# Vchitect/Latte

Measured on NVIDIA H100. Metric: denoising-steps/sec Latte-XL/2 16x256x256 (CFG pair per step), higher is better.
Workload: dtype fp16

## Files before the change

latte_b200/csrc/gemm.cu:

```cuda
#include <cstdio>
#include "common.h"
#include "ptx.cuh"
#include "wgmma.cuh"

#include <cstdlib>

namespace b200 {

namespace {

constexpr int BM = 128;
constexpr int BK = 64;
constexpr int kThreads = 384;
constexpr int kProducerRegs = 40;
constexpr int kConsumerRegs = 232;

template <int BN, int EPI>
struct Cfg {
  static constexpr bool RESID = EPI == B200_EPI_GATE_RESIDUAL;
  static constexpr int A_BYTES = BM * BK * 2;
  static constexpr int B_BYTES = BN * BK * 2;
  static constexpr int STAGE_BYTES = A_BYTES + B_BYTES;
  static constexpr int BAR_BYTES = 256;
  static constexpr int STAGES_FIT = (232448 - BAR_BYTES - 1024) / STAGE_BYTES;
  static constexpr int STAGES = STAGES_FIT > 8 ? 8 : STAGES_FIT;
  static constexpr int BAR_OFF = STAGES * STAGE_BYTES;
  static constexpr int SMEM_BYTES = BAR_OFF + BAR_BYTES + 1024;
  static_assert(STAGE_BYTES % 1024 == 0, "stage must keep 1 KiB alignment");
  static_assert(SMEM_BYTES <= 232448, "exceeds the 227 KB per-CTA shared memory limit");
  static_assert(2 * STAGES <= BAR_BYTES / 8, "barrier area too small");
};

struct GemmDev {
  int M, N, K;
  int num_m, num_n;
  const float* bias;
  void* out16;
  const float* gate;
  long long gate_bs;
  int rows_per_batch;
  const float* row_add;
  int row_add_div, row_add_period;
  const uint16_t* add16;
  uint16_t* out16b;
  int conv_taps, conv_cblk, conv_h, conv_w, conv_bw, conv_bh;
  int conv_dx[9], conv_dy[9], conv_dz[9];
  float* resid;
  int streamk;
  unsigned long long* sk_flags;
};

__device__ __forceinline__ void flag_release(unsigned long long* f, unsigned long long v) {
  asm volatile("st.release.gpu.global.u64 [%0], %1;" ::"l"(f), "l"(v) : "memory");
}
__device__ __forceinline__ void flag_wait(const unsigned long long* f, unsigned long long want) {
  const long long t0 = clock64();
  while (true) {
    unsigned long long v;
    asm volatile("ld.acquire.gpu.global.u64 %0, [%1];" : "=l"(v) : "l"(f) : "memory");
    if (v == want) return;
    if (clock64() - t0 > 4000000000LL) __trap();
    __nanosleep(64);
  }
// ... 18 lines not shown
  __host__ __device__ bool next(int& tile, int& kb0, int& kb1) {
    if (wave < full_waves) {
      tile = wave * P + pair;
      ++wave;
      kb0 = 0;
      kb1 = num_kb;
      return tile < num_tiles;
    }
    if (u >= u_end) return false;
    const int t = static_cast<int>((u_end - 1) / num_kb);
    const long long t0 = static_cast<long long>(t) * num_kb;
    kb1 = static_cast<int>(u_end - t0);
    kb0 = u > t0 ? static_cast<int>(u - t0) : 0;
    tile = full_waves * P + t;
    u_end = t0 + kb0;
    return true;
  }
};

__device__ __forceinline__ float gelu_tanh_grad(float x) {
  const float k0 = 0.7978845608028654f, k1 = 0.044715f;
  const float x2 = x * x;
  float t;
  asm("tanh.approx.f32 %0, %1;" : "=f"(t) : "f"(k0 * fmaf(k1 * x2, x, x)));
  const float sech2 = fmaf(-t, t, 1.0f);
  return fmaf(0.5f * x * sech2, k0 * fmaf(3.0f * k1, x2, 1.0f), fmaf(0.5f, t, 0.5f));
}

__device__ __forceinline__ float resid_delta(float acc, float b, float gt, float ra, bool has_ra) {
  const float dv = __fmul_rn(gt, __fadd_rn(acc, b));
  return has_ra ? __fadd_rn(dv, ra) : dv;
}

constexpr int kEpiChunk = 8;
__device__ __forceinline__ void epi_chunk_fence() { __syncwarp(); }

__device__ __forceinline__ float gelu_tanh(float x) {
  const float u = 0.7978845608028654f * fmaf(0.044715f * x * x, x, x);
  float t;
  asm("tanh.approx.f32 %0, %1;" : "=f"(t) : "f"(u));
  const float hx = 0.5f * x;
  return fmaf(hx, t, hx);
}

template <int BN, int EPI, bool BF16, int MN>
__global__ void __cluster_dims__(2, 1, 1) __launch_bounds__(kThreads, 1)
gemm_kernel(const __grid_constant__ CUtensorMap tmA, const __grid_constant__ CUtensorMap tmB, const GemmDev p) {
  using C = Cfg<BN, EPI>;
  constexpr int TA = MN & 1, TB = MN >> 1;
  static_assert(MN == 0 || MN == 2 || MN == 3, "operand layouts: 0 forward, 2 dgrad, 3 wgrad");
  static_assert((BN / 8) % kEpiChunk == 0, "the epilogue chunks must tile the 8-column groups of a tile exactly");
  extern __shared__ uint8_t smem_raw[];
  uint8_t* smem = reinterpret_cast<uint8_t*>((reinterpret_cast<uintptr_t>(smem_raw) + 1023) & ~uintptr_t(1023));
  uint64_t* bars = reinterpret_cast<uint64_t*>(smem + C::BAR_OFF);
  uint64_t* full = bars;
  uint64_t* empty = bars + C::STAGES;

  const int warp = threadIdx.x >> 5;
  const int lane = threadIdx.x & 31;

  if (threadIdx.x == 0) {
    tma_prefetch_desc(&tmA);
    tma_prefetch_desc(&tmB);
    for (int i = 0; i < C::STAGES; ++i) {
      mbar_init(&full[i], 1);
      mbar_init(&empty[i], 4);
    }
    fence_mbar_init();
  }
  cluster_sync_all();
  pdl_launch_dependents();

  const uint32_t rank = cluster_ctarank();
  const int num_pair_m = (p.num_m + 1) / 2;
  const int num_tiles = num_pair_m * p.num_n;
  const int my_pair = blockIdx.x >> 1;
  const int num_pairs = gridDim.x >> 1;
  const int num_kb = p.K / BK;
  const bool streamk = C::RESID && p.streamk != 0;

  if (warp < 4) {
    setmaxnreg_dec<kProducerRegs>();
    if (threadIdx.x == 0) {
      pdl_wait();
      TileSched sched(my_pair, num_pairs, num_tiles, num_kb, streamk);
      int stage = 0;
      uint32_t phase = 0;
      int tile, kb0, kb1;
      while (sched.next(tile, kb0, kb1)) {
        const int m_blk = 2 * (tile / p.num_n) + static_cast<int>(rank), n_blk = tile % p.num_n;
        const int w_row0 = n_blk * BN + static_cast<int>(rank) * (BN / 2);
        for (int kb = kb0; kb < kb1; ++kb) {
          mbar_wait(&empty[stage], phase ^ 1);
          mbar_arrive_expect_tx(&full[stage], C::STAGE_BYTES);
          uint8_t* sa = smem + stage * C::STAGE_BYTES;
          if (MN == 0 && p.conv_taps > 0) {
// ... 2 lines not shown
            const int hw = p.conv_h * p.conv_w;
            const int img = pix0 / hw, rem = pix0 % hw;
            tma_load_4d(sa, &tmA, &full[stage], cb * BK, rem % p.conv_w + p.conv_dx[tap], rem / p.conv_w + p.conv_dy[tap],
                        img + p.conv_dz[tap]);
          } else if constexpr (TA) {
#pragma unroll
            for (int j = 0; j < BM / 64; ++j) tma_load_2d(sa + j * 8192, &tmA, &full[stage], m_blk * BM + j * 64, kb * BK);
          } else {
            tma_load_2d(sa, &tmA, &full[stage], kb * BK, m_blk * BM);
          }
          if constexpr (TB) {
            constexpr int per_cta = BN / 128;
#pragma unroll
            for (int j = 0; j < per_cta; ++j)
              tma_load_2d_mcast(sa + C::A_BYTES + (rank * per_cta + j) * 8192, &tmB, &full[stage], w_row0 + j * 64, kb * BK, 0x3);
          } else {
            tma_load_2d_mcast(sa + C::A_BYTES + rank * (C::B_BYTES / 2), &tmB, &full[stage], kb * BK, w_row0, 0x3);
          }
          if (++stage == C::STAGES) { stage = 0; phase ^= 1; }
        }
      }
    }
    __syncwarp();
  } else {
    setmaxnreg_inc<kConsumerRegs>();
    pdl_wait();
    const int wg = (warp >> 2) - 1;
    const int te = threadIdx.x & 127;
    const int w4 = te >> 5, g = lane >> 2, cq = lane & 3;
    const uint32_t empty_peer = mapa_u32(&empty[0], rank ^ 1u);
    int stage = 0;
    uint32_t phase = 0;
    float acc[BN / 2];
    TileSched sched(my_pair, num_pairs, num_tiles, num_kb, streamk);
    int tile, kb0, kb1;
    while (sched.next(tile, kb0, kb1)) {
      const int m0 = (2 * (tile / p.num_n) + static_cast<int>(rank)) * BM, n0 = (tile % p.num_n) * BN;
      int prev = -1;
      for (int kb = kb0; kb < kb1; ++kb) {
        mbar_wait(&full[stage], phase);
        const uint32_t sa = smem_u32(smem + stage * C::STAGE_BYTES), sb = sa + C::A_BYTES;
        wgmma_fence();
        const uint64_t da = gmma_desc(sa + wg * 8192, TA ? 8192 : 16, 1024, GMMA_LAYOUT_SW128);
        const uint64_t db = gmma_desc(sb, TB ? 8192 : 16, 1024, GMMA_LAYOUT_SW128);
#pragma unroll
        for (int k = 0; k < BK / 16; ++k)
          WgmmaSS<BN, TA, TB, BF16>::mma(acc, gmma_desc_advance(da, k * (TA ? 2048 : 32)),
                                         gmma_desc_advance(db, k * (TB ? 2048 : 32)), (kb != kb0 || k) ? 1u : 0u);
        wgmma_commit();
        wgmma_wait<1>();
        if (prev >= 0 && te == 0) {
          mbar_arrive(&empty[prev]);
          mbar_arrive_cluster(empty_peer + prev * 8);
        }
        prev = stage;
        if (++stage == C::STAGES) { stage = 0; phase ^= 1; }
      }
      wgmma_wait<0>();
      reg_fence(acc);
      if (te == 0) {
        mbar_arrive(&empty[prev]);
        mbar_arrive_cluster(empty_peer + prev * 8);
      }

      const int r0 = m0 + wg * 64 + w4 * 16 + g;
      if constexpr (C::RESID) {
        const bool first_seg = kb0 == 0;
        const bool partial = kb0 > 0 || kb1 < num_kb;
        unsigned long long* flag = nullptr;
        if (partial) flag = p.sk_flags + (static_cast<size_t>(tile - sched.full_waves * num_pairs) * 2 + rank) * 2 + wg;
        if (kb0 > 0) {
          if (te == 0) {
            flag_wait(flag, static_cast<unsigned long long>(kb0));
            if (kb1 == num_kb) flag_release(flag, 0ull);
          }
          asm volatile("bar.sync %0, 128;" ::"r"(1 + wg) : "memory");
        }
        const float* bias = (p.bias && first_seg) ? p.bias : nullptr;
        const int live = (p.N - n0) / 8 < BN / 8 ? (p.N - n0) / 8 : BN / 8;
#pragma unroll
        for (int h = 0; h < 2; ++h) {
          const int row = r0 + 8 * h;
          const bool row_ok = row < p.M;
          if (BN > 192 && !row_ok) continue;
          const int prow = row_ok ? row : p.M - 1;
          const float* gate_row = p.gate + static_cast<long long>(prow / p.rows_per_batch) * p.gate_bs;
          const float* add_row = (p.row_add && first_seg) ? p.row_add + static_cast<size_t>((prow / p.row_add_div) % p.row_add_period) * p.N : nullptr;
          float* xrow = p.resid + static_cast<size_t>(prow) * p.N;
          if (BN <= 192 && live == BN / 8) {
#pragma unroll
            for (int j0 = 0; j0 < BN / 8; j0 += kEpiChunk) {
              float2 x[kEpiChunk];
#pragma unroll
              for (int j = 0; j < kEpiChunk; ++j)
                if (row_ok) x[j] = *reinterpret_cast<const float2*>(xrow + n0 + 8 * (j0 + j) + 2 * cq);
#pragma unroll
              for (int j = 0; j < kEpiChunk; ++j) {
                if (!row_ok) continue;
                const int col = n0 + 8 * (j0 + j) + 2 * cq;
                const float2 b2 = bias ? __ldg(reinterpret_cast<const float2*>(bias + col)) : make_float2(0.f, 0.f);
                const float2 gt = __ldg(reinterpret_cast<const float2*>(gate_row + col));
                const float2 ra = add_row ? __ldg(reinterpret_cast<const float2*>(add_row + col)) : make_float2(0.f, 0.f);
                x[j].x = __fadd_rn(x[j].x, resid_delta(acc[4 * (j0 + j) + 2 * h], b2.x, gt.x, ra.x, add_row != nullptr));
                x[j].y = __fadd_rn(x[j].y, resid_delta(acc[4 * (j0 + j) + 2 * h + 1], b2.y, gt.y, ra.y, add_row != nullptr));
                *reinterpret_cast<float2*>(xrow + col) = x[j];
              }
              epi_chunk_fence();
            }
          } else if (row_ok) {
#pragma unroll
            for (int j = 0; j < BN / 8; ++j) {
              if (j >= live) break;
              const int col = n0 + 8 * j + 2 * cq;
              const float2 b2 = bias ? __ldg(reinterpret_cast<const float2*>(bias + col)) : make_float2(0.f, 0.f);
              const float2 gt = __ldg(reinterpret_cast<const float2*>(gate_row + col));
              const float2 ra = add_row ? __ldg(reinterpret_cast<const float2*>(add_row + col)) : make_float2(0.f, 0.f);
              float2 x = *reinterpret_cast<const float2*>(xrow + col);
              x.x = __fadd_rn(x.x, resid_delta(acc[4 * j + 2 * h], b2.x, gt.x, ra.x, add_row != nullptr));
              x.y = __fadd_rn(x.y, resid_delta(acc[4 * j + 2 * h + 1], b2.y, gt.y, ra.y, add_row != nullptr));
              *reinterpret_cast<float2*>(xrow + col) = x;
            }
          }
        }
        if (partial && kb1 < num_kb) {
          __threadfence();
          asm volatile("bar.sync %0, 128;" ::"r"(1 + wg) : "memory");
          if (te == 0) flag_release(flag, static_cast<unsigned long long>(kb1));
        }
      } else {
        bool done = false;
        if constexpr (EPI == B200_EPI_BIAS || EPI == B200_EPI_BIAS_GELU) {
          if (p.N - n0 >= BN) {
            const bool row_ok[2] = {r0 < p.M, r0 + 8 < p.M};
            uint32_t* orow[2];
#pragma unroll
            for (int h = 0; h < 2; ++h)
              orow[h] = reinterpret_cast<uint32_t*>(reinterpret_cast<uint16_t*>(p.out16) + static_cast<size_t>(r0 + 8 * h) * p.N);
#pragma unroll
            for (int j0 = 0; j0 < BN / 8; j0 += kEpiChunk) {
              float2 b[kEpiChunk];
#pragma unroll
              for (int j = 0; j < kEpiChunk; ++j)
                b[j] = p.bias ? __ldg(reinterpret_cast<const float2*>(p.bias + n0 + 8 * (j0 + j) + 2 * cq)) : make_float2(0.f, 0.f);
#pragma unroll
              for (int h = 0; h < 2; ++h) {
                if (!row_ok[h]) continue;
#pragma unroll
                for (int j = 0; j < kEpiChunk; ++j) {
                  const int col = n0 + 8 * (j0 + j) + 2 * cq;
                  float f0 = acc[4 * (j0 + j) + 2 * h], f1 = acc[4 * (j0 + j) + 2 * h + 1];
                  if (p.bias) { f0 += b[j].x; f1 += b[j].y; }
                  if constexpr (EPI == B200_EPI_BIAS_GELU) { f0 = gelu_tanh(f0); f1 = gelu_tanh(f1); }
                  orow[h][col / 2] = pack2<BF16>(f0, f1);
                }
              }
              epi_chunk_fence();
            }
            done = true;
          }
        }
        if (!done) {
#pragma unroll
          for (int h = 0; h < 2; ++h) {
            const int row = r0 + 8 * h;
            if (row >= p.M) continue;
            uint32_t* orow = reinterpret_cast<uint32_t*>(reinterpret_cast<uint16_t*>(p.out16) + static_cast<size_t>(row) * p.N);
            const int live = (p.N - n0) / 8 < BN / 8 ? (p.N - n0) / 8 : BN / 8;
#pragma unroll
            for (int j = 0; j < BN / 8; ++j) {
              if (j >= live) break;
              const int col = n0 + 8 * j + 2 * cq;
              float f0 = acc[4 * j + 2 * h], f1 = acc[4 * j + 2 * h + 1];
              if (p.bias) {
                const float2 b = __ldg(reinterpret_cast<const float2*>(p.bias + col));
                f0 += b.x; f1 += b.y;
              }
              if constexpr (EPI == B200_EPI_BIAS_GELU) { f0 = gelu_tanh(f0); f1 = gelu_tanh(f1); }
              uint32_t val = pack2<BF16>(f0, f1);
              const size_t off = (static_cast<size_t>(row) * p.N + col) / 2;
              if constexpr (EPI == B200_EPI_BIAS_MUL16) {
                const float2 a = unpack2<BF16>(val), r = unpack2<BF16>(__ldg(reinterpret_cast<const uint32_t*>(p.add16) + off));
                val = pack2<BF16>(a.x * r.x, a.y * r.y);
              }
              if constexpr (EPI == B200_EPI_MUL_GELUGRAD16) {
                const float2 a = unpack2<BF16>(val), r = unpack2<BF16>(__ldg(reinterpret_cast<const uint32_t*>(p.add16) + off));
                val = pack2<BF16>(a.x * gelu_tanh_grad(r.x), a.y * gelu_tanh_grad(r.y));
              }
              if constexpr (EPI == B200_EPI_BIAS_GELU_BOTH) {
                const float2 a = unpack2<BF16>(val);
                reinterpret_cast<uint32_t*>(p.out16b)[off] = pack2<BF16>(gelu_tanh(a.x), gelu_tanh(a.y));
              }
              if constexpr (EPI == B200_EPI_BIAS_ADD16) {
                const float2 a = unpack2<BF16>(val), r = unpack2<BF16>(__ldg(reinterpret_cast<const uint32_t*>(p.add16) + off));
                val = pack2<BF16>(a.x + r.x, a.y + r.y);
              }
              orow[col / 2] = val;
            }
          }
        }
      }
    }
  }

  cluster_sync_all();
}

template <int BN, int EPI, bool BF16, int MN>
int launch_one(const CUtensorMap& tmA, const CUtensorMap& tmB, const GemmDev& p, int grid, cudaStream_t stream) {
  using C = Cfg<BN, EPI>;
  auto kern = gemm_kernel<BN, EPI, BF16, MN>;
  B200_SET_SMEM_ONCE(kern, C::SMEM_BYTES);
  B200_CHECK_CUDA(launch_pdl(kern, dim3(grid), dim3(kThreads), C::SMEM_BYTES, stream, tmA, tmB, p));
  return B200_OK;
}

template <int BN, bool BF16>
int launch_epi(int epi, int mn, const CUtensorMap& tmA, const CUtensorMap& tmB, const GemmDev& p, int grid, cudaStream_t s) {
  if (mn == 0) {
    switch (epi) {
      case B200_EPI_BIAS: return launch_one<BN, B200_EPI_BIAS, BF16, 0>(tmA, tmB, p, grid, s);
      case B200_EPI_BIAS_GELU: return launch_one<BN, B200_EPI_BIAS_GELU, BF16, 0>(tmA, tmB, p, grid, s);
      case B200_EPI_GATE_RESIDUAL: return launch_one<BN, B200_EPI_GATE_RESIDUAL, BF16, 0>(tmA, tmB, p, grid, s);
      case B200_EPI_BIAS_ADD16: return launch_one<BN, B200_EPI_BIAS_ADD16, BF16, 0>(tmA, tmB, p, grid, s);
      case B200_EPI_BIAS_MUL16: return launch_one<BN, B200_EPI_BIAS_MUL16, BF16, 0>(tmA, tmB, p, grid, s);
      case B200_EPI_BIAS_GELU_BOTH: return launch_one<BN, B200_EPI_BIAS_GELU_BOTH, BF16, 0>(tmA, tmB, p, grid, s);
      case B200_EPI_MUL_GELUGRAD16: return launch_one<BN, B200_EPI_MUL_GELUGRAD16, BF16, 0>(tmA, tmB, p, grid, s);
    }
  }
  if constexpr (BN != 192) {
    if (mn == 2 && epi == B200_EPI_BIAS) return launch_one<BN, B200_EPI_BIAS, BF16, 2>(tmA, tmB, p, grid, s);
    if (mn == 2 && epi == B200_EPI_MUL_GELUGRAD16) return launch_one<BN, B200_EPI_MUL_GELUGRAD16, BF16, 2>(tmA, tmB, p, grid, s);
    if (mn == 3 && epi == B200_EPI_GATE_RESIDUAL) return launch_one<BN, B200_EPI_GATE_RESIDUAL, BF16, 3>(tmA, tmB, p, grid, s);
  }
  set_error("gemm: epilogue %d with operand layout %d and block_n %d is not built", epi, mn, BN);
  return B200_ERR_UNSUPPORTED;
}

template <int BN>
int launch_bn(int bf16, int epi, int mn, const CUtensorMap& tmA, const CUtensorMap& tmB, const GemmDev& p, int grid,
              cudaStream_t s) {
  return bf16 ? launch_epi<BN, true>(epi, mn, tmA, tmB, p, grid, s) : launch_epi<BN, false>(epi, mn, tmA, tmB, p, grid, s);
}

constexpr int kStreamKMinKb = 32;
constexpr int kSkFlags = B200_GEMM_SK_FLAGS;

int streamk_min_kb() {
  static const int v = env_int("B200_GEMM_SK_MINKB", kStreamKMinKb);
  return v;
}


int pick_block_n(int M, int N, int K, bool resid, int sms) {
  if (N <= 128) return 128;
  static const bool no_sk = env_int("B200_GEMM_NO_STREAMK", 0) != 0;
  const bool sk = resid && !no_sk && K / BK >= streamk_min_kb();
  const int cand[3] = {256, 192, 128};
  int best = 128;
  double best_cost = 1e300;
  for (int i = 0; i < 3; ++i) {
    const long long tiles = static_cast<long long>((M + BM - 1) / BM) * ((N + cand[i] - 1) / cand[i]);
    const double waves = (sk && tiles > sms) ? static_cast<double>(tiles) / sms : static_cast<double>((tiles + sms - 1) / sms);
    const double cost = waves * (128 + cand[i] / 2);
    if (cost < best_cost - 1e-9) { best_cost = cost; best = cand[i]; }
  }
  return best;
}

struct GemmPlan { int bn, pairs, pair_tiles, num_kb, streamk; };
GemmPlan plan_gemm(int M, int N, int K, bool resid, int block_n, int sms, bool split_small = false) {
  static const bool no_sk = env_int("B200_GEMM_NO_STREAMK", 0) != 0;
  GemmPlan g;
  g.bn = block_n ? block_n : pick_block_n(M, N, K, resid, sms);
  const int num_m = (M + BM - 1) / BM, num_n = (N + g.bn - 1) / g.bn;
// ... 57 lines not shown
  const bool resid = a.epilogue == B200_EPI_GATE_RESIDUAL;
  if (resid) {
    B200_REQUIRE(a.resid && a.gate && a.rows_per_batch > 0, B200_ERR_SHAPE, "gemm: gated-residual epilogue needs resid, gate, rows_per_batch");
    B200_REQUIRE((reinterpret_cast<uintptr_t>(a.resid) & 15) == 0 && (reinterpret_cast<uintptr_t>(a.gate) & 15) == 0 &&
                     (a.gate_batch_stride % 4) == 0,
                 B200_ERR_ALIGN, "gemm: resid/gate must be 16-byte aligned");
    B200_REQUIRE(!a.row_add || (reinterpret_cast<uintptr_t>(a.row_add) & 15) == 0, B200_ERR_ALIGN, "gemm: row_add must be 16-byte aligned");
  } else {
    B200_REQUIRE(a.out16 && (reinterpret_cast<uintptr_t>(a.out16) & 15) == 0, B200_ERR_ALIGN, "gemm: out16 must be 16-byte aligned");
  }
  B200_REQUIRE(!a.bias || (reinterpret_cast<uintptr_t>(a.bias) & 15) == 0, B200_ERR_ALIGN, "gemm: bias must be 16-byte aligned");
  B200_TRY(check_arch());
  int sms = 0;
  B200_TRY(device_sm_count(&sms));

  B200_REQUIRE(a.block_n == 0 || a.block_n == 128 || a.block_n == 192 || a.block_n == 256, B200_ERR_UNSUPPORTED,
               "gemm: block_n must be 128, 192 or 256 (got %d)", a.block_n);
  int block_n = a.block_n;
  if (a.mn_major) {
    B200_REQUIRE((a.mn_major == 2 || a.mn_major == 3) && a.conv_taps == 0 && (!(a.mn_major & 1) || a.M % 8 == 0) &&
                     (!(a.mn_major & 2) || a.N % 128 == 0) && (a.block_n == 0 || a.block_n == 128 || a.block_n == 256),
                 B200_ERR_UNSUPPORTED, "gemm (transposed operands): mn_major 2 or 3, M %% 8 == 0, N %% 128 == 0, block_n 128 or 256 (M=%d N=%d)",
                 a.M, a.N);
    if (block_n == 0) {
      block_n = pick_block_n(a.M, a.N, a.K, a.epilogue == B200_EPI_GATE_RESIDUAL, sms);
      if (block_n == 192) block_n = (a.N % 256 == 0 || a.N > 1024) ? 256 : 128;
      static const int wgrad_bn = env_int("B200_WGRAD_BN", 0);
      if (a.mn_major == 3) block_n = (wgrad_bn == 128 || wgrad_bn == 256) ? wgrad_bn : (a.N >= 256 ? 256 : block_n);
    }
  }
  const GemmPlan plan = plan_gemm(a.M, a.N, a.K, a.epilogue == B200_EPI_GATE_RESIDUAL, block_n, sms, a.mn_major == 3);
  const int bn = plan.bn;

  CUtensorMap tmA, tmB;
  int conv_bw = 0, conv_bh = 0;
  {
    if (a.conv_taps > 0) {
      B200_REQUIRE(a.conv_taps <= 9 && a.conv_c % BK == 0 && a.K == a.conv_taps * a.conv_c &&
                       a.M == a.conv_n * a.conv_h * a.conv_w,
                   B200_ERR_SHAPE, "conv: inconsistent geometry (taps %d, C %d, K %d, M %d)", a.conv_taps, a.conv_c, a.K, a.M);
      conv_bw = a.conv_w >= BM ? BM : a.conv_w;
      conv_bh = BM / conv_bw;
      B200_REQUIRE(BM % conv_bw == 0 && a.conv_w % conv_bw == 0 && a.conv_h % conv_bh == 0, B200_ERR_UNSUPPORTED,
                   "conv: %dx%d feature map cannot be tiled by 128-pixel patches", a.conv_h, a.conv_w);
      const uint64_t dimsA[4] = {static_cast<uint64_t>(a.conv_c), static_cast<uint64_t>(a.conv_w), static_cast<uint64_t>(a.conv_h),
                                 static_cast<uint64_t>(a.conv_n)};
      const uint64_t strA[3] = {static_cast<uint64_t>(a.conv_c) * 2, static_cast<uint64_t>(a.conv_c) * 2 * a.conv_w,
                                static_cast<uint64_t>(a.conv_c) * 2 * a.conv_w * a.conv_h};
      const uint32_t boxA[4] = {BK, static_cast<uint32_t>(conv_bw), static_cast<uint32_t>(conv_bh), 1};
      B200_TRY(make_tmap_16bit(&tmA, a.A, 4, dimsA, strA, boxA, TMAP_SW_128));
    } else if (a.mn_major & 1) {
      const uint64_t dimsA[2] = {static_cast<uint64_t>(a.M), static_cast<uint64_t>(a.K)};
      const uint64_t strA[1] = {static_cast<uint64_t>(a.M) * 2};
      const uint32_t boxA[2] = {64, BK};
      B200_TRY(make_tmap_16bit(&tmA, a.A, 2, dimsA, strA, boxA, TMAP_SW_128));
    } else {
      const uint64_t dimsA[2] = {static_cast<uint64_t>(a.K), static_cast<uint64_t>(a.M)};
      const uint64_t strA[1] = {static_cast<uint64_t>(a.K) * 2};
      const uint32_t boxA[2] = {BK, BM};
      B200_TRY(make_tmap_16bit(&tmA, a.A, 2, dimsA, strA, boxA, TMAP_SW_128));
    }
    if (a.mn_major & 2) {
      const uint64_t dimsB[2] = {static_cast<uint64_t>(a.N), static_cast<uint64_t>(a.K)};
      const uint64_t strB[1] = {static_cast<uint64_t>(a.N) * 2};
      const uint32_t boxB[2] = {64, BK};
      B200_TRY(make_tmap_16bit(&tmB, a.W, 2, dimsB, strB, boxB, TMAP_SW_128));
    } else {
      const uint64_t dimsB[2] = {static_cast<uint64_t>(a.K), static_cast<uint64_t>(a.N)};
      const uint64_t strB[1] = {static_cast<uint64_t>(a.K) * 2};
      const uint32_t boxB[2] = {BK, static_cast<uint32_t>(bn / 2)};
      B200_TRY(make_tmap_16bit(&tmB, a.W, 2, dimsB, strB, boxB, TMAP_SW_128));
    }
  }
  GemmDev p;
  p.M = a.M; p.N = a.N; p.K = a.K;
  p.num_m = (a.M + BM - 1) / BM;
  p.num_n = (a.N + bn - 1) / bn;
  p.bias = a.bias;
  p.out16 = a.out16;
  p.gate = a.gate;
  p.gate_bs = a.gate_batch_stride;
  p.rows_per_batch = a.rows_per_batch > 0 ? a.rows_per_batch : 1;
  p.row_add = a.row_add;
  p.row_add_div = a.row_add_div > 0 ? a.row_add_div : 1;
  p.row_add_period = a.row_add_period > 0 ? a.row_add_period : 1;
  p.add16 = static_cast<const uint16_t*>(a.add16);
  p.out16b = static_cast<uint16_t*>(a.out16b);
  p.conv_taps = a.conv_taps;
  p.conv_cblk = a.conv_taps > 0 ? a.conv_c / BK : 0;
  p.conv_h = a.conv_h; p.conv_w = a.conv_w; p.conv_bw = conv_bw; p.conv_bh = conv_bh;
  for (int i = 0; i < 9; ++i) { p.conv_dx[i] = a.conv_dx[i]; p.conv_dy[i] = a.conv_dy[i]; p.conv_dz[i] = a.conv_dz[i]; }
  p.resid = a.resid;
  const int pair_tiles = plan.pair_tiles;
  const int grid = 2 * plan.pairs;
  {
    const int pairs = plan.pairs;
    const int streamed = pair_tiles % pairs + pairs;
    p.streamk = (plan.streamk && a.sk_flags != nullptr && streamed * 4 <= kSkFlags) ? 1 : 0;
    p.sk_flags = p.streamk ? a.sk_flags : nullptr;
  }
  switch (bn) {
    case 128: return launch_bn<128>(a.bf16, a.epilogue, a.mn_major, tmA, tmB, p, grid, stream);
    case 192: return launch_bn<192>(a.bf16, a.epilogue, a.mn_major, tmA, tmB, p, grid, stream);
    default: return launch_bn<256>(a.bf16, a.epilogue, a.mn_major, tmA, tmB, p, grid, stream);
  }
}

}
```

latte_b200/csrc/ptx.cuh:

```cuda
#pragma once
#include <cuda.h>
#include <cuda_runtime.h>
#include <cuda_fp16.h>
#include <cuda_bf16.h>
#include <cstdint>
#include <cstdio>

namespace b200 {

#ifndef B200_HANG_CYCLES
#define B200_HANG_CYCLES (4000000000ll)
#endif

__device__ __forceinline__ uint32_t smem_u32(const void* p) {
  return static_cast<uint32_t>(__cvta_generic_to_shared(p));
}
__device__ __forceinline__ uint32_t lane_id() { return threadIdx.x & 31; }

__device__ __forceinline__ void pdl_wait() { asm volatile("griddepcontrol.wait;" ::: "memory"); }
__device__ __forceinline__ void pdl_launch_dependents() { asm volatile("griddepcontrol.launch_dependents;" ::: "memory"); }

__device__ __forceinline__ void mbar_init(uint64_t* bar, uint32_t count) {
  asm volatile("mbarrier.init.shared::cta.b64 [%0], %1;" ::"r"(smem_u32(bar)), "r"(count) : "memory");
}
// ... 42 lines not shown
    }
  }
}

__device__ __forceinline__ bool mbar_try_wait_cluster(uint64_t* bar, uint32_t parity) {
  uint32_t ok;
  asm volatile(
      "{\n\t.reg .pred p;\n\t"
      "mbarrier.try_wait.parity.acquire.cluster.shared::cta.b64 p, [%1], %2;\n\t"
      "selp.u32 %0, 1, 0, p;\n\t}"
      : "=r"(ok)
      : "r"(smem_u32(bar)), "r"(parity)
      : "memory");
  return ok != 0;
}
__device__ __forceinline__ void mbar_wait_cluster(uint64_t* bar, uint32_t parity) {
  if (mbar_try_wait_cluster(bar, parity)) return;
  long long t0 = clock64();
  while (!mbar_try_wait_cluster(bar, parity)) {
    if (clock64() - t0 > B200_HANG_CYCLES) {
      __trap();
    }
  }
}

template <uint32_t N>
__device__ __forceinline__ void setmaxnreg_dec() { asm volatile("setmaxnreg.dec.sync.aligned.u32 %0;" ::"n"(N)); }
template <uint32_t N>
__device__ __forceinline__ void setmaxnreg_inc() { asm volatile("setmaxnreg.inc.sync.aligned.u32 %0;" ::"n"(N)); }

__device__ __forceinline__ void fence_proxy_async_smem() {
  asm volatile("fence.proxy.async.shared::cta;" ::: "memory");
}

__device__ __forceinline__ void tma_prefetch_desc(const CUtensorMap* m) {
  asm volatile("prefetch.tensormap [%0];" ::"l"(reinterpret_cast<uint64_t>(m)) : "memory");
}
__device__ __forceinline__ void tma_load_2d(void* dst, const CUtensorMap* m, uint64_t* bar, int c0, int c1) {
  asm volatile(
      "cp.async.bulk.tensor.2d.shared::cluster.global.tile.mbarrier::complete_tx::bytes [%0], [%1, {%3, %4}], [%2];"
      ::"r"(smem_u32(dst)), "l"(reinterpret_cast<uint64_t>(m)), "r"(smem_u32(bar)), "r"(c0), "r"(c1)
      : "memory");
}
__device__ __forceinline__ void tma_load_3d(void* dst, const CUtensorMap* m, uint64_t* bar, int c0, int c1, int c2) {
  asm volatile(
      "cp.async.bulk.tensor.3d.shared::cluster.global.tile.mbarrier::complete_tx::bytes [%0], [%1, {%3, %4, %5}], [%2];"
      ::"r"(smem_u32(dst)), "l"(reinterpret_cast<uint64_t>(m)), "r"(smem_u32(bar)), "r"(c0), "r"(c1), "r"(c2)
      : "memory");
}
__device__ __forceinline__ void tma_load_4d(void* dst, const CUtensorMap* m, uint64_t* bar, int c0, int c1, int c2,
                                            int c3) {
  asm volatile(
      "cp.async.bulk.tensor.4d.shared::cluster.global.tile.mbarrier::complete_tx::bytes [%0], [%1, {%3, %4, %5, %6}], [%2];"
      ::"r"(smem_u32(dst)), "l"(reinterpret_cast<uint64_t>(m)), "r"(smem_u32(bar)), "r"(c0), "r"(c1), "r"(c2), "r"(c3)
      : "memory");
}

__device__ __forceinline__ void tma_load_2d_mcast(void* dst, const CUtensorMap* m, uint64_t* bar, int c0, int c1,
                                                  uint16_t mask) {
  asm volatile(
      "cp.async.bulk.tensor.2d.shared::cluster.global.tile.mbarrier::complete_tx::bytes.multicast::cluster"
      " [%0], [%1, {%3, %4}], [%2], %5;"
      ::"r"(smem_u32(dst)), "l"(reinterpret_cast<uint64_t>(m)), "r"(smem_u32(bar)), "r"(c0), "r"(c1), "h"(mask)
      : "memory");
}

// ... 3 lines not shown
  return r;
}
__device__ __forceinline__ void mbar_arrive_cluster(uint32_t bar_cluster_addr) {
  asm volatile("mbarrier.arrive.shared::cluster.b64 _, [%0];" ::"r"(bar_cluster_addr) : "memory");
}
__device__ __forceinline__ uint32_t cluster_ctarank() {
  uint32_t r;
  asm volatile("mov.u32 %0, %%cluster_ctarank;" : "=r"(r));
  return r;
}
__device__ __forceinline__ void cluster_sync_all() {
  asm volatile("barrier.cluster.arrive.release.aligned;\n\tbarrier.cluster.wait.acquire.aligned;" ::: "memory");
}

__device__ __forceinline__ void tma_store_2d(const CUtensorMap* m, const void* src, int c0, int c1) {
  asm volatile("cp.async.bulk.tensor.2d.global.shared::cta.bulk_group [%0, {%2, %3}], [%1];"
               ::"l"(reinterpret_cast<uint64_t>(m)), "r"(smem_u32(src)), "r"(c0), "r"(c1)
               : "memory");
}
__device__ __forceinline__ void tma_store_3d(const CUtensorMap* m, const void* src, int c0, int c1, int c2) {
  asm volatile("cp.async.bulk.tensor.3d.global.shared::cta.bulk_group [%0, {%2, %3, %4}], [%1];"
               ::"l"(reinterpret_cast<uint64_t>(m)), "r"(smem_u32(src)), "r"(c0), "r"(c1), "r"(c2)
               : "memory");
}
__device__ __forceinline__ void tma_store_4d(const CUtensorMap* m, const void* src, int c0, int c1, int c2, int c3) {
  asm volatile("cp.async.bulk.tensor.4d.global.shared::cta.bulk_group [%0, {%2, %3, %4, %5}], [%1];"
               ::"l"(reinterpret_cast<uint64_t>(m)), "r"(smem_u32(src)), "r"(c0), "r"(c1), "r"(c2), "r"(c3)
               : "memory");
}
__device__ __forceinline__ void tma_reduce_add_2d(const CUtensorMap* m, const void* src, int c0, int c1) {
  asm volatile("cp.reduce.async.bulk.tensor.2d.global.shared::cta.add.tile.bulk_group [%0, {%2, %3}], [%1];"
               ::"l"(reinterpret_cast<uint64_t>(m)), "r"(smem_u32(src)), "r"(c0), "r"(c1)
               : "memory");
}
__device__ __forceinline__ void tma_store_commit() { asm volatile("cp.async.bulk.commit_group;" ::: "memory"); }
template <int N>
__device__ __forceinline__ void tma_store_wait_read() {
  asm volatile("cp.async.bulk.wait_group.read %0;" ::"n"(N) : "memory");
}
template <int N>
__device__ __forceinline__ void tma_store_wait_all() {
  asm volatile("cp.async.bulk.wait_group %0;" ::"n"(N) : "memory");
}

enum : uint32_t { GMMA_LAYOUT_NONE = 0, GMMA_LAYOUT_SW128 = 1, GMMA_LAYOUT_SW64 = 2, GMMA_LAYOUT_SW32 = 3 };

__device__ __forceinline__ uint64_t gmma_desc(uint32_t saddr, uint32_t lbo_bytes, uint32_t sbo_bytes, uint32_t layout) {
  uint64_t d = 0;
  d |= static_cast<uint64_t>((saddr >> 4) & 0x3FFF);
  d |= static_cast<uint64_t>((lbo_bytes >> 4) & 0x3FFF) << 16;
  d |= static_cast<uint64_t>((sbo_bytes >> 4) & 0x3FFF) << 32;
  d |= static_cast<uint64_t>(layout) << 62;
  return d;
}
__device__ __forceinline__ uint64_t gmma_desc_advance(uint64_t desc, uint32_t bytes) {
  return desc + static_cast<uint64_t>(bytes >> 4);
}
__device__ __forceinline__ void wgmma_fence() { asm volatile("wgmma.fence.sync.aligned;" ::: "memory"); }
__device__ __forceinline__ void wgmma_commit() { asm volatile("wgmma.commit_group.sync.aligned;" ::: "memory"); }
template <int N>
__device__ __forceinline__ void wgmma_wait() { asm volatile("wgmma.wait_group.sync.aligned %0;" ::"n"(N) : "memory"); }
template <int N>
__device__ __forceinline__ void reg_fence(float (&d)[N]) {
#pragma unroll
  for (int i = 0; i < N; ++i) asm volatile("" : "+f"(d[i])::"memory");
}
// ... 22 lines not shown
```

Baseline: 39.48.

## Stage GEMM epilogues through swizzled shared memory and TMA store/reduce-add

Replaces the per-thread direct global stores in the GEMM epilogue with staging into double-buffered 128B-swizzled shared memory (stmatrix for 16-bit outputs, st.shared for fp32 residual deltas). The tile is then written out by a TMA bulk store, or by a TMA reduce-add into the fp32 residual stream instead of a read-modify-write. The aim is coalesced, asynchronous output traffic and removal of the residual read. In exchange, 32 KB of shared memory goes to epilogue buffers, which can cut pipeline stages. It also adds two named barriers per chunk and changes stream-K ordering to rely on async-proxy fences.

```diff
diff --git a/latte_b200/csrc/gemm.cu b/latte_b200/csrc/gemm.cu
--- a/latte_b200/csrc/gemm.cu
+++ b/latte_b200/csrc/gemm.cu
@@ -14,6 +14,8 @@
 constexpr int kThreads = 384;
 constexpr int kProducerRegs = 40;
 constexpr int kConsumerRegs = 232;
+
+constexpr int kEpiBufBytes = 64 * 128;
 
 template <int BN, int EPI>
 struct Cfg {
@@ -21,14 +23,17 @@
   static constexpr int A_BYTES = BM * BK * 2;
   static constexpr int B_BYTES = BN * BK * 2;
   static constexpr int STAGE_BYTES = A_BYTES + B_BYTES;
+  static constexpr int EPI_BYTES = 2 * 2 * kEpiBufBytes;
   static constexpr int BAR_BYTES = 256;
-  static constexpr int STAGES_FIT = (232448 - BAR_BYTES - 1024) / STAGE_BYTES;
+  static constexpr int STAGES_FIT = (232448 - EPI_BYTES - BAR_BYTES - 1024) / STAGE_BYTES;
   static constexpr int STAGES = STAGES_FIT > 8 ? 8 : STAGES_FIT;
-  static constexpr int BAR_OFF = STAGES * STAGE_BYTES;
+  static constexpr int EPI_OFF = STAGES * STAGE_BYTES;
+  static constexpr int BAR_OFF = EPI_OFF + EPI_BYTES;
   static constexpr int SMEM_BYTES = BAR_OFF + BAR_BYTES + 1024;
   static_assert(STAGE_BYTES % 1024 == 0, "stage must keep 1 KiB alignment");
   static_assert(SMEM_BYTES <= 232448, "exceeds the 227 KB per-CTA shared memory limit");
   static_assert(2 * STAGES <= BAR_BYTES / 8, "barrier area too small");
+  static_assert(BN % 64 == 0, "the 16-bit epilogue works in 64-column chunks");
 };
 
 struct GemmDev {
@@ -113,8 +118,7 @@
   return has_ra ? __fadd_rn(dv, ra) : dv;
 }
 
-constexpr int kEpiChunk = 8;
-__device__ __forceinline__ void epi_chunk_fence() { __syncwarp(); }
+__device__ __forceinline__ void epi_bar(int wg) { asm volatile("bar.sync %0, 128;" ::"r"(1 + wg) : "memory"); }
 
 __device__ __forceinline__ float gelu_tanh(float x) {
   const float u = 0.7978845608028654f * fmaf(0.044715f * x * x, x, x);
@@ -126,11 +130,11 @@
 
 template <int BN, int EPI, bool BF16, int MN>
 __global__ void __cluster_dims__(2, 1, 1) __launch_bounds__(kThreads, 1)
-gemm_kernel(const __grid_constant__ CUtensorMap tmA, const __grid_constant__ CUtensorMap tmB, const GemmDev p) {
+gemm_kernel(const __grid_constant__ CUtensorMap tmA, const __grid_constant__ CUtensorMap tmB,
+            const __grid_constant__ CUtensorMap tmC, const __grid_constant__ CUtensorMap tmC2, const GemmDev p) {
   using C = Cfg<BN, EPI>;
   constexpr int TA = MN & 1, TB = MN >> 1;
   static_assert(MN == 0 || MN == 2 || MN == 3, "operand layouts: 0 forward, 2 dgrad, 3 wgrad");
-  static_assert((BN / 8) % kEpiChunk == 0, "the epilogue chunks must tile the 8-column groups of a tile exactly");
   extern __shared__ uint8_t smem_raw[];
   uint8_t* smem = reinterpret_cast<uint8_t*>((reinterpret_cast<uintptr_t>(smem_raw) + 1023) & ~uintptr_t(1023));
   uint64_t* bars = reinterpret_cast<uint64_t*>(smem + C::BAR_OFF);
@@ -143,6 +147,8 @@
   if (threadIdx.x == 0) {
     tma_prefetch_desc(&tmA);
     tma_prefetch_desc(&tmB);
+    tma_prefetch_desc(&tmC);
+    if constexpr (EPI == B200_EPI_BIAS_GELU_BOTH) tma_prefetch_desc(&tmC2);
     for (int i = 0; i < C::STAGES; ++i) {
       mbar_init(&full[i], 1);
       mbar_init(&empty[i], 4);
@@ -211,6 +217,8 @@
     int stage = 0;
     uint32_t phase = 0;
     float acc[BN / 2];
+    uint8_t* epi = smem + C::EPI_OFF;
+    int ep = 0;
     TileSched sched(my_pair, num_pairs, num_tiles, num_kb, streamk);
     int tile, kb0, kb1;
     while (sched.next(tile, kb0, kb1)) {
@@ -242,183 +250,160 @@
         mbar_arrive_cluster(empty_peer + prev * 8);
       }
 
-      const int r0 = m0 + wg * 64 + w4 * 16 + g;
+      const int m0w = m0 + wg * 64;
+      const int lr0 = w4 * 16 + g;
       if constexpr (C::RESID) {
         const bool first_seg = kb0 == 0;
         const bool partial = kb0 > 0 || kb1 < num_kb;
         unsigned long long* flag = nullptr;
         if (partial) flag = p.sk_flags + (static_cast<size_t>(tile - sched.full_waves * num_pairs) * 2 + rank) * 2 + wg;
-        if (kb0 > 0) {
-          if (te == 0) {
-            flag_wait(flag, static_cast<unsigned long long>(kb0));
-            if (kb1 == num_kb) flag_release(flag, 0ull);
-          }
-          asm volatile("bar.sync %0, 128;" ::"r"(1 + wg) : "memory");
+        bool ordered = kb0 == 0;
+        const float* bias = (p.bias && first_seg) ? p.bias : nullptr;
+        const float* gate_row[2];
+        const float* add_row[2];
+#pragma unroll
+        for (int h = 0; h < 2; ++h) {
+          const int row = m0w + lr0 + 8 * h < p.M ? m0w + lr0 + 8 * h : p.M - 1;
+          gate_row[h] = p.gate + static_cast<long long>(row / p.rows_per_batch) * p.gate_bs;
+          add_row[h] = (p.row_add && first_seg) ? p.row_add + static_cast<size_t>((row / p.row_add_div) % p.row_add_period) * p.N : nullptr;
         }
-        const float* bias = (p.bias && first_seg) ? p.bias : nullptr;
-        const int live = (p.N - n0) / 8 < BN / 8 ? (p.N - n0) / 8 : BN / 8;
-#pragma unroll
-        for (int h = 0; h < 2; ++h) {
-          const int row = r0 + 8 * h;
-          const bool row_ok = row < p.M;
-          if (BN > 192 && !row_ok) continue;
-          const int prow = row_ok ? row : p.M - 1;
-          const float* gate_row = p.gate + static_cast<long long>(prow / p.rows_per_batch) * p.gate_bs;
-          const float* add_row = (p.row_add && first_seg) ? p.row_add + static_cast<size_t>((prow / p.row_add_div) % p.row_add_period) * p.N : nullptr;
-          float* xrow = p.resid + static_cast<size_t>(prow) * p.N;
-          if (BN <= 192 && live == BN / 8) {
-#pragma unroll
-            for (int j0 = 0; j0 < BN / 8; j0 += kEpiChunk) {
-              float2 x[kEpiChunk];
-#pragma unroll
-              for (int j = 0; j < kEpiChunk; ++j)
-                if (row_ok) x[j] = *reinterpret_cast<const float2*>(xrow + n0 + 8 * (j0 + j) + 2 * cq);
-#pragma unroll
-              for (int j = 0; j < kEpiChunk; ++j) {
-                if (!row_ok) continue;
-                const int col = n0 + 8 * (j0 + j) + 2 * cq;
-                const float2 b2 = bias ? __ldg(reinterpret_cast<const float2*>(bias + col)) : make_float2(0.f, 0.f);
-                const float2 gt = __ldg(reinterpret_cast<const float2*>(gate_row + col));
-                const float2 ra = add_row ? __ldg(reinterpret_cast<const float2*>(add_row + col)) : make_float2(0.f, 0.f);
-                x[j].x = __fadd_rn(x[j].x, resid_delta(acc[4 * (j0 + j) + 2 * h], b2.x, gt.x, ra.x, add_row != nullptr));
-                x[j].y = __fadd_rn(x[j].y, resid_delta(acc[4 * (j0 + j) + 2 * h + 1], b2.y, gt.y, ra.y, add_row != nullptr));
-                *reinterpret_cast<float2*>(xrow + col) = x[j];
-              }
-              epi_chunk_fence();
-            }
-          } else if (row_ok) {
-#pragma unroll
-            for (int j = 0; j < BN / 8; ++j) {
-              if (j >= live) break;
-              const int col = n0 + 8 * j + 2 * cq;
-              const float2 b2 = bias ? __ldg(reinterpret_cast<const float2*>(bias + col)) : make_float2(0.f, 0.f);
-              const float2 gt = __ldg(reinterpret_cast<const float2*>(gate_row + col));
-              const float2 ra = add_row ? __ldg(reinterpret_cast<const float2*>(add_row + col)) : make_float2(0.f, 0.f);
-              float2 x = *reinterpret_cast<const float2*>(xrow + col);
-              x.x = __fadd_rn(x.x, resid_delta(acc[4 * j + 2 * h], b2.x, gt.x, ra.x, add_row != nullptr));
-              x.y = __fadd_rn(x.y, resid_delta(acc[4 * j + 2 * h + 1], b2.y, gt.y, ra.y, add_row != nullptr));
-              *reinterpret_cast<float2*>(xrow + col) = x;
+#pragma unroll
+        for (int c = 0; c < BN / 32; ++c) {
+          if (n0 + 32 * c >= p.N) break;
+          uint8_t* buf = epi + (2 * wg + (ep & 1)) * kEpiBufBytes;
+          const uint32_t buf_addr = smem_u32(buf);
+#pragma unroll
+          for (int jj = 0; jj < 4; ++jj) {
+            const int j = 4 * c + jj, col = n0 + 8 * j + 2 * cq;
+            const float2 b2 = bias ? __ldg(reinterpret_cast<const float2*>(bias + col)) : make_float2(0.f, 0.f);
+#pragma unroll
+            for (int h = 0; h < 2; ++h) {
+              const float2 gt = __ldg(reinterpret_cast<const float2*>(gate_row[h] + col));
+              const float2 ra = add_row[h] ? __ldg(reinterpret_cast<const float2*>(add_row[h] + col)) : make_float2(0.f, 0.f);
+              const float d0 = resid_delta(acc[4 * j + 2 * h], b2.x, gt.x, ra.x, add_row[h] != nullptr);
+              const float d1 = resid_delta(acc[4 * j + 2 * h + 1], b2.y, gt.y, ra.y, add_row[h] != nullptr);
+              st_shared_f2(buf_addr + (lr0 + 8 * h) * 128 + (((2 * jj + (cq >> 1)) ^ g) << 4) + 8 * (cq & 1), d0, d1);
             }
           }
+          fence_proxy_async_smem();
+          epi_bar(wg);
+          if (te == 0) {
+            if (!ordered) {
+              flag_wait(flag, static_cast<unsigned long long>(kb0));
+              fence_proxy_async_global();
+              if (kb1 == num_kb) flag_release(flag, 0ull);
+              ordered = true;
+            }
+            tma_reduce_add_2d(&tmC, buf, n0 + 32 * c, m0w);
+            tma_store_commit();
+            tma_store_wait_read<1>();
+          }
+          epi_bar(wg);
+          ++ep;
         }
-        if (partial && kb1 < num_kb) {
-          __threadfence();
-          asm volatile("bar.sync %0, 128;" ::"r"(1 + wg) : "memory");
-          if (te == 0) flag_release(flag, static_cast<unsigned long long>(kb1));
+        if (partial && kb1 < num_kb && te == 0) {
+          tma_store_wait_all<0>();
+          fence_proxy_async_global();
+          flag_release(flag, static_cast<unsigned long long>(kb1));
         }
       } else {
-        bool done = false;
-        if constexpr (EPI == B200_EPI_BIAS || EPI == B200_EPI_BIAS_GELU) {
-          if (p.N - n0 >= BN) {
-            const bool row_ok[2] = {r0 < p.M, r0 + 8 < p.M};
-            uint32_t* orow[2];
-#pragma unroll
-            for (int h = 0; h < 2; ++h)
-              orow[h] = reinterpret_cast<uint32_t*>(reinterpret_cast<uint16_t*>(p.out16) + static_cast<size_t>(r0 + 8 * h) * p.N);
-#pragma unroll
-            for (int j0 = 0; j0 < BN / 8; j0 += kEpiChunk) {
-              float2 b[kEpiChunk];
-#pragma unroll
-              for (int j = 0; j < kEpiChunk; ++j)
-                b[j] = p.bias ? __ldg(reinterpret_cast<const float2*>(p.bias + n0 + 8 * (j0 + j) + 2 * cq)) : make_float2(0.f, 0.f);
+        constexpr bool TWO = EPI == B200_EPI_BIAS_GELU_BOTH;
+        const int mi = lane >> 3;
+        const int lrow = w4 * 16 + (lane & 7) + 8 * (mi & 1);
+#pragma unroll
+        for (int c = 0; c < BN / 64; ++c) {
+          if (n0 + 64 * c >= p.N) break;
+          uint8_t* buf = epi + (2 * wg + (TWO ? 0 : (ep & 1))) * kEpiBufBytes;
+          const uint32_t row_addr = smem_u32(buf) + lrow * 128;
+#pragma unroll
+          for (int jp = 0; jp < 4; ++jp) {
+            uint32_t v[4], vb[4];
+#pragma unroll
+            for (int q = 0; q < 2; ++q) {
+              const int j = 8 * c + 2 * jp + q, col = n0 + 8 * j + 2 * cq;
+              const bool col_ok = col < p.N;
+              const float2 b2 = (p.bias && col_ok) ? __ldg(reinterpret_cast<const float2*>(p.bias + col)) : make_float2(0.f, 0.f);
 #pragma unroll
               for (int h = 0; h < 2; ++h) {
-                if (!row_ok[h]) continue;
-#pragma unroll
-                for (int j = 0; j < kEpiChunk; ++j) {
-                  const int col = n0 + 8 * (j0 + j) + 2 * cq;
-                  float f0 = acc[4 * (j0 + j) + 2 * h], f1 = acc[4 * (j0 + j) + 2 * h + 1];
-                  if (p.bias) { f0 += b[j].x; f1 += b[j].y; }
-                  if constexpr (EPI == B200_EPI_BIAS_GELU) { f0 = gelu_tanh(f0); f1 = gelu_tanh(f1); }
-                  orow[h][col / 2] = pack2<BF16>(f0, f1);
+                float f0 = acc[4 * j + 2 * h], f1 = acc[4 * j + 2 * h + 1];
+                if (p.bias) { f0 += b2.x; f1 += b2.y; }
+                if constexpr (EPI == B200_EPI_BIAS_GELU) { f0 = gelu_tanh(f0); f1 = gelu_tanh(f1); }
+                uint32_t val = pack2<BF16>(f0, f1);
+                if constexpr (EPI == B200_EPI_BIAS_ADD16 || EPI == B200_EPI_BIAS_MUL16 || EPI == B200_EPI_MUL_GELUGRAD16) {
+                  const int row = m0w + lr0 + 8 * h;
+                  const uint32_t side = (row < p.M && col_ok)
+                      ? __ldg(reinterpret_cast<const uint32_t*>(p.add16) + (static_cast<size_t>(row) * p.N + col) / 2) : 0u;
+                  const float2 a = unpack2<BF16>(val), r = unpack2<BF16>(side);
+                  if constexpr (EPI == B200_EPI_BIAS_ADD16) val = pack2<BF16>(a.x + r.x, a.y + r.y);
+                  if constexpr (EPI == B200_EPI_BIAS_MUL16) val = pack2<BF16>(a.x * r.x, a.y * r.y);
+                  if constexpr (EPI == B200_EPI_MUL_GELUGRAD16) val = pack2<BF16>(a.x * gelu_tanh_grad(r.x), a.y * gelu_tanh_grad(r.y));
                 }
+                if constexpr (TWO) {
+                  const float2 a = unpack2<BF16>(val);
+                  vb[2 * q + h] = pack2<BF16>(gelu_tanh(a.x), gelu_tanh(a.y));
+                }
+                v[2 * q + h] = val;
               }
-              epi_chunk_fence();
             }
-            done = true;
+            const uint32_t unit = ((2 * jp + (mi >> 1)) ^ (lane & 7)) << 4;
+            stmatrix_x4(row_addr + unit, v[0], v[1], v[2], v[3]);
+            if constexpr (TWO) stmatrix_x4(row_addr + kEpiBufBytes + unit, vb[0], vb[1], vb[2], vb[3]);
           }
-        }
-        if (!done) {
-#pragma unroll
-          for (int h = 0; h < 2; ++h) {
-            const int row = r0 + 8 * h;
-            if (row >= p.M) continue;
-            uint32_t* orow = reinterpret_cast<uint32_t*>(reinterpret_cast<uint16_t*>(p.out16) + static_cast<size_t>(row) * p.N);
-            const int live = (p.N - n0) / 8 < BN / 8 ? (p.N - n0) / 8 : BN / 8;
-#pragma unroll
-            for (int j = 0; j < BN / 8; ++j) {
-              if (j >= live) break;
-              const int col = n0 + 8 * j + 2 * cq;
-              float f0 = acc[4 * j + 2 * h], f1 = acc[4 * j + 2 * h + 1];
-              if (p.bias) {
-                const float2 b = __ldg(reinterpret_cast<const float2*>(p.bias + col));
-                f0 += b.x; f1 += b.y;
-              }
-              if constexpr (EPI == B200_EPI_BIAS_GELU) { f0 = gelu_tanh(f0); f1 = gelu_tanh(f1); }
-              uint32_t val = pack2<BF16>(f0, f1);
-              const size_t off = (static_cast<size_t>(row) * p.N + col) / 2;
-              if constexpr (EPI == B200_EPI_BIAS_MUL16) {
-                const float2 a = unpack2<BF16>(val), r = unpack2<BF16>(__ldg(reinterpret_cast<const uint32_t*>(p.add16) + off));
-                val = pack2<BF16>(a.x * r.x, a.y * r.y);
-              }
-              if constexpr (EPI == B200_EPI_MUL_GELUGRAD16) {
-                const float2 a = unpack2<BF16>(val), r = unpack2<BF16>(__ldg(reinterpret_cast<const uint32_t*>(p.add16) + off));
-                val = pack2<BF16>(a.x * gelu_tanh_grad(r.x), a.y * gelu_tanh_grad(r.y));
-              }
-              if constexpr (EPI == B200_EPI_BIAS_GELU_BOTH) {
-                const float2 a = unpack2<BF16>(val);
-                reinterpret_cast<uint32_t*>(p.out16b)[off] = pack2<BF16>(gelu_tanh(a.x), gelu_tanh(a.y));
-              }
-              if constexpr (EPI == B200_EPI_BIAS_ADD16) {
-                const float2 a = unpack2<BF16>(val), r = unpack2<BF16>(__ldg(reinterpret_cast<const uint32_t*>(p.add16) + off));
-                val = pack2<BF16>(a.x + r.x, a.y + r.y);
-              }
-              orow[col / 2] = val;
-            }
+          fence_proxy_async_smem();
+          epi_bar(wg);
+          if (te == 0) {
+            tma_store_2d(&tmC, buf, n0 + 64 * c, m0w);
+            if constexpr (TWO) tma_store_2d(&tmC2, buf + kEpiBufBytes, n0 + 64 * c, m0w);
+            tma_store_commit();
+            if constexpr (TWO) tma_store_wait_read<0>(); else tma_store_wait_read<1>();
           }
+          epi_bar(wg);
+          ++ep;
         }
       }
     }
+    if (te == 0) tma_store_wait_all<0>();
   }
 
   cluster_sync_all();
 }
 
+struct GemmMaps { CUtensorMap a, b, c, c2; };
+
 template <int BN, int EPI, bool BF16, int MN>
-int launch_one(const CUtensorMap& tmA, const CUtensorMap& tmB, const GemmDev& p, int grid, cudaStream_t stream) {
+int launch_one(const GemmMaps& tm, const GemmDev& p, int grid, cudaStream_t stream) {
   using C = Cfg<BN, EPI>;
   auto kern = gemm_kernel<BN, EPI, BF16, MN>;
   B200_SET_SMEM_ONCE(kern, C::SMEM_BYTES);
-  B200_CHECK_CUDA(launch_pdl(kern, dim3(grid), dim3(kThreads), C::SMEM_BYTES, stream, tmA, tmB, p));
+  B200_CHECK_CUDA(launch_pdl(kern, dim3(grid), dim3(kThreads), C::SMEM_BYTES, stream, tm.a, tm.b, tm.c, tm.c2, p));
   return B200_OK;
 }
 
 template <int BN, bool BF16>
-int launch_epi(int epi, int mn, const CUtensorMap& tmA, const CUtensorMap& tmB, const GemmDev& p, int grid, cudaStream_t s) {
+int launch_epi(int epi, int mn, const GemmMaps& tm, const GemmDev& p, int grid, cudaStream_t s) {
   if (mn == 0) {
     switch (epi) {
-      case B200_EPI_BIAS: return launch_one<BN, B200_EPI_BIAS, BF16, 0>(tmA, tmB, p, grid, s);
-      case B200_EPI_BIAS_GELU: return launch_one<BN, B200_EPI_BIAS_GELU, BF16, 0>(tmA, tmB, p, grid, s);
-      case B200_EPI_GATE_RESIDUAL: return launch_one<BN, B200_EPI_GATE_RESIDUAL, BF16, 0>(tmA, tmB, p, grid, s);
-      case B200_EPI_BIAS_ADD16: return launch_one<BN, B200_EPI_BIAS_ADD16, BF16, 0>(tmA, tmB, p, grid, s);
-      case B200_EPI_BIAS_MUL16: return launch_one<BN, B200_EPI_BIAS_MUL16, BF16, 0>(tmA, tmB, p, grid, s);
-      case B200_EPI_BIAS_GELU_BOTH: return launch_one<BN, B200_EPI_BIAS_GELU_BOTH, BF16, 0>(tmA, tmB, p, grid, s);
-      case B200_EPI_MUL_GELUGRAD16: return launch_one<BN, B200_EPI_MUL_GELUGRAD16, BF16, 0>(tmA, tmB, p, grid, s);
+      case B200_EPI_BIAS: return launch_one<BN, B200_EPI_BIAS, BF16, 0>(tm, p, grid, s);
+      case B200_EPI_BIAS_GELU: return launch_one<BN, B200_EPI_BIAS_GELU, BF16, 0>(tm, p, grid, s);
+      case B200_EPI_GATE_RESIDUAL: return launch_one<BN, B200_EPI_GATE_RESIDUAL, BF16, 0>(tm, p, grid, s);
+      case B200_EPI_BIAS_ADD16: return launch_one<BN, B200_EPI_BIAS_ADD16, BF16, 0>(tm, p, grid, s);
+      case B200_EPI_BIAS_MUL16: return launch_one<BN, B200_EPI_BIAS_MUL16, BF16, 0>(tm, p, grid, s);
+      case B200_EPI_BIAS_GELU_BOTH: return launch_one<BN, B200_EPI_BIAS_GELU_BOTH, BF16, 0>(tm, p, grid, s);
+      case B200_EPI_MUL_GELUGRAD16: return launch_one<BN, B200_EPI_MUL_GELUGRAD16, BF16, 0>(tm, p, grid, s);
     }
   }
   if constexpr (BN != 192) {
-    if (mn == 2 && epi == B200_EPI_BIAS) return launch_one<BN, B200_EPI_BIAS, BF16, 2>(tmA, tmB, p, grid, s);
-    if (mn == 2 && epi == B200_EPI_MUL_GELUGRAD16) return launch_one<BN, B200_EPI_MUL_GELUGRAD16, BF16, 2>(tmA, tmB, p, grid, s);
-    if (mn == 3 && epi == B200_EPI_GATE_RESIDUAL) return launch_one<BN, B200_EPI_GATE_RESIDUAL, BF16, 3>(tmA, tmB, p, grid, s);
+    if (mn == 2 && epi == B200_EPI_BIAS) return launch_one<BN, B200_EPI_BIAS, BF16, 2>(tm, p, grid, s);
+    if (mn == 2 && epi == B200_EPI_MUL_GELUGRAD16) return launch_one<BN, B200_EPI_MUL_GELUGRAD16, BF16, 2>(tm, p, grid, s);
+    if (mn == 3 && epi == B200_EPI_GATE_RESIDUAL) return launch_one<BN, B200_EPI_GATE_RESIDUAL, BF16, 3>(tm, p, grid, s);
   }
   set_error("gemm: epilogue %d with operand layout %d and block_n %d is not built", epi, mn, BN);
   return B200_ERR_UNSUPPORTED;
 }
 
 template <int BN>
-int launch_bn(int bf16, int epi, int mn, const CUtensorMap& tmA, const CUtensorMap& tmB, const GemmDev& p, int grid,
-              cudaStream_t s) {
-  return bf16 ? launch_epi<BN, true>(epi, mn, tmA, tmB, p, grid, s) : launch_epi<BN, false>(epi, mn, tmA, tmB, p, grid, s);
+int launch_bn(int bf16, int epi, int mn, const GemmMaps& tm, const GemmDev& p, int grid, cudaStream_t s) {
+  return bf16 ? launch_epi<BN, true>(epi, mn, tm, p, grid, s) : launch_epi<BN, false>(epi, mn, tm, p, grid, s);
 }
 
 constexpr int kStreamKMinKb = 32;
@@ -542,7 +527,9 @@
   const GemmPlan plan = plan_gemm(a.M, a.N, a.K, a.epilogue == B200_EPI_GATE_RESIDUAL, block_n, sms, a.mn_major == 3);
   const int bn = plan.bn;
 
-  CUtensorMap tmA, tmB;
+  GemmMaps tm;
+  CUtensorMap& tmA = tm.a;
+  CUtensorMap& tmB = tm.b;
   int conv_bw = 0, conv_bh = 0;
   {
     if (a.conv_taps > 0) {
@@ -581,6 +568,19 @@
       const uint32_t boxB[2] = {BK, static_cast<uint32_t>(bn / 2)};
       B200_TRY(make_tmap_16bit(&tmB, a.W, 2, dimsB, strB, boxB, TMAP_SW_128));
     }
+    const uint64_t dimsC[2] = {static_cast<uint64_t>(a.N), static_cast<uint64_t>(a.M)};
+    if (resid) {
+      const uint64_t strC[1] = {static_cast<uint64_t>(a.N) * 4};
+      const uint32_t boxC[2] = {32, 64};
+      B200_TRY(make_tmap(&tm.c, a.resid, 4, 2, dimsC, strC, boxC, TMAP_SW_128));
+      tm.c2 = tm.c;
+    } else {
+      const uint64_t strC[1] = {static_cast<uint64_t>(a.N) * 2};
+      const uint32_t boxC[2] = {64, 64};
+      B200_TRY(make_tmap_16bit(&tm.c, a.out16, 2, dimsC, strC, boxC, TMAP_SW_128));
+      if (a.epilogue == B200_EPI_BIAS_GELU_BOTH) B200_TRY(make_tmap_16bit(&tm.c2, a.out16b, 2, dimsC, strC, boxC, TMAP_SW_128));
+      else tm.c2 = tm.c;
+    }
   }
   GemmDev p;
   p.M = a.M; p.N = a.N; p.K = a.K;
@@ -610,10 +610,10 @@
     p.sk_flags = p.streamk ? a.sk_flags : nullptr;
   }
   switch (bn) {
-    case 128: return launch_bn<128>(a.bf16, a.epilogue, a.mn_major, tmA, tmB, p, grid, stream);
-    case 192: return launch_bn<192>(a.bf16, a.epilogue, a.mn_major, tmA, tmB, p, grid, stream);
-    default: return launch_bn<256>(a.bf16, a.epilogue, a.mn_major, tmA, tmB, p, grid, stream);
-  }
-}
-
-}
+    case 128: return launch_bn<128>(a.bf16, a.epilogue, a.mn_major, tm, p, grid, stream);
+    case 192: return launch_bn<192>(a.bf16, a.epilogue, a.mn_major, tm, p, grid, stream);
+    default: return launch_bn<256>(a.bf16, a.epilogue, a.mn_major, tm, p, grid, stream);
+  }
+}
+
+}
diff --git a/latte_b200/csrc/ptx.cuh b/latte_b200/csrc/ptx.cuh
--- a/latte_b200/csrc/ptx.cuh
+++ b/latte_b200/csrc/ptx.cuh
@@ -98,6 +98,7 @@
 __device__ __forceinline__ void fence_proxy_async_smem() {
   asm volatile("fence.proxy.async.shared::cta;" ::: "memory");
 }
+__device__ __forceinline__ void fence_proxy_async_global() { asm volatile("fence.proxy.async.global;" ::: "memory"); }
 
 __device__ __forceinline__ void tma_prefetch_desc(const CUtensorMap* m) {
   asm volatile("prefetch.tensormap [%0];" ::"l"(reinterpret_cast<uint64_t>(m)) : "memory");
@@ -167,6 +168,13 @@
   asm volatile("cp.reduce.async.bulk.tensor.2d.global.shared::cta.add.tile.bulk_group [%0, {%2, %3}], [%1];"
                ::"l"(reinterpret_cast<uint64_t>(m)), "r"(smem_u32(src)), "r"(c0), "r"(c1)
                : "memory");
+}
+__device__ __forceinline__ void st_shared_f2(uint32_t saddr, float a, float b) {
+  asm volatile("st.shared.v2.f32 [%0], {%1, %2};" ::"r"(saddr), "f"(a), "f"(b) : "memory");
+}
+__device__ __forceinline__ void stmatrix_x4(uint32_t saddr, uint32_t r0, uint32_t r1, uint32_t r2, uint32_t r3) {
+  asm volatile("stmatrix.sync.aligned.m8n8.x4.shared.b16 [%0], {%1, %2, %3, %4};"
+               ::"r"(saddr), "r"(r0), "r"(r1), "r"(r2), "r"(r3) : "memory");
 }
 __device__ __forceinline__ void tma_store_commit() { asm volatile("cp.async.bulk.commit_group;" ::: "memory"); }
 template <int N>
```

New measurement: 46.69, median of 6. 18.3% higher.
